# eth-cscs/conflux

Hardware: NVIDIA H100
Metric: LU GFLOP/s (FP64, (2/3)N^3) (higher is better)
Workload: dtype f64

## Files before the change

### conflux_b200/__init__.py

```python
import ctypes

import numpy as np

from ._lib import ConfluxError, LIB_PATH, SYMBOLS, ShareLayout, check, lib

__all__ = ["pinned_empty", "pinned_free", "Comm", "lu_params", "LU_rep", "LU_rep_fixed", "rbt_multipliers", "LU_rep_rbt", "lu_rbt_solve", "lu_rbt_apply_local", "residual", "validate", "lu_solve", "lu_rcond", "lu_refine", "lu_refine_x", "lu_equilibrate", "lu_svx", "lu_equilibrate_b", "lu_svxx", "lu_inverse", "lu_det", "rhs_local_cols", "lu_solve_local", "timeline", "auto_grid", "lu_dims", "init_matrix_host", "ConfluxError", "dbg", "cholesky", "chol_dims", "chol_auto_grid"]


def auto_grid(M, N, P):
    px, py, pz = ctypes.c_int(), ctypes.c_int(), ctypes.c_int()
    check(lib().cflx_auto_grid(int(M), int(N), int(P), ctypes.byref(px), ctypes.byref(py), ctypes.byref(pz)), "auto_grid")
    return px.value, py.value, pz.value


def lu_dims(M, N, v, Px, Py, Pz):
    o = (ctypes.c_int * 8)()
    check(lib().cflx_lu_dims(int(M), int(N), int(v), int(Px), int(Py), int(Pz), o), "lu_dims")
    return dict(M=o[0], N=o[1], Ml=o[2], Nl=o[3], Nt=o[4], nlayr=o[5], Mt=o[6], P=o[7])


def init_matrix_host(M, N, v, Px, Py, Pz, rank, seed=42, out=None):
    d = lu_dims(M, N, v, Px, Py, Pz)
    if out is None:
        out = np.empty((d["Ml"], d["Nl"]), dtype=np.float64)
# ... 816 lines not shown
                                 ctypes.byref(exp), ctypes.byref(neg), ctypes.byref(fz), ctypes.byref(nf)), "dbg_det")
        return dict(mantissa=mant.value, exponent=exp.value, neg=neg.value, first_zero=fz.value, nonfinite=nf.value)

    @staticmethod
    def panel(P, reps=1):
        P = np.ascontiguousarray(P, dtype=np.float64)
        n, v = P.shape
        perm = np.zeros(v, dtype=np.int32)
        A00 = np.zeros((v, v))
        LU = np.zeros((max(n, 1), v))
        ms = ctypes.c_double()
        check(lib().cflx_dbg_panel(n, v, P.ctypes.data, perm.ctypes.data, A00.ctypes.data, LU.ctypes.data, int(reps),
                                   ctypes.byref(ms)), "dbg_panel")
        return perm, A00, LU[:n], ms.value

    @staticmethod
    def trsm(A00, B=None, R=None, nb=0, ld=0):
        A00 = np.ascontiguousarray(A00, dtype=np.float64)
        v = A00.shape[0]
        X = Y = None
        n = B.shape[0] if B is not None else R.shape[1]
        if B is not None:
            B = np.ascontiguousarray(B, dtype=np.float64)
            X = np.empty_like(B)
        if R is not None:
            R = np.ascontiguousarray(R, dtype=np.float64)
            Y = np.empty_like(R)
        check(lib().cflx_dbg_trsm(n, v, int(nb), int(ld), A00.ctypes.data, B.ctypes.data if B is not None else None,
                                  X.ctypes.data if X is not None else None, R.ctypes.data if R is not None else None,
                                  Y.ctypes.data if Y is not None else None), "dbg_trsm")
        return X, Y

    @staticmethod
    def diag_inverse(A00, nb):
        A00 = np.ascontiguousarray(A00, dtype=np.float64)
        v = A00.shape[0]
        Uinv = np.empty((max(v // nb, 1), nb, nb))
        LinvT = np.empty_like(Uinv)
        check(lib().cflx_dbg_diag_inverse(v, int(nb), A00.ctypes.data, Uinv.ctypes.data, LinvT.ctypes.data), "dbg_diag_inverse")
        return Uinv, LinvT

    @staticmethod
    def potrf_tile(A, variant=0):
        A = np.ascontiguousarray(A, dtype=np.float64)
        v = A.shape[0]
        L = np.empty((v, v))
        LT = np.empty((v, v))
        info = ctypes.c_int()
        check(lib().cflx_dbg_potrf_tile(v, A.ctypes.data, L.ctypes.data, LT.ctypes.data, ctypes.byref(info), int(variant)),
              "dbg_potrf_tile")
        return L, LT, info.value

    @staticmethod
    def getrf_nopiv_tile(A, tiny=0.0, variant=0):
        A = np.ascontiguousarray(A, dtype=np.float64)
        v = A.shape[0]
        LU = np.empty((v, v))
        nrepl, info = ctypes.c_int(), ctypes.c_int()
        check(lib().cflx_dbg_getrf_nopiv_tile(v, A.ctypes.data, float(tiny), LU.ctypes.data, ctypes.byref(nrepl),
                                              ctypes.byref(info), int(variant)), "dbg_getrf_nopiv_tile")
        return LU, nrepl.value, info.value

    @staticmethod
    def ozaki_gemm(AT, B, C=None, reps=1, want_planes=False, row0=0, col0=0, max_ctas=0):
        AT = np.ascontiguousarray(AT, dtype=np.float64)
        B = np.ascontiguousarray(B, dtype=np.float64)
# ... 43 lines not shown
```

### conflux_b200/_lib.py

```python
import ctypes
import os

_HERE = os.path.dirname(os.path.abspath(__file__))
LIB_PATH = os.path.join(_HERE, "libconflux_b200.so")
_lib = None

c_double_p = ctypes.POINTER(ctypes.c_double)
c_int_p = ctypes.POINTER(ctypes.c_int)


class ConfluxError(RuntimeError):
    pass


class ShareLayout(ctypes.Structure):
    _fields_ = [(f, ctypes.c_int) for f in ("M", "v", "Kappa", "Ml", "Nl", "Px", "Py", "pi", "pj")]


SYMBOLS = [
    "cflx_last_error", "cflx_version", "cflx_device_count", "cflx_get_unique_id", "cflx_comm_create",
    "cflx_comm_barrier", "cflx_comm_destroy", "cflx_host_alloc", "cflx_host_free", "cflx_auto_grid", "cflx_lu_dims", "cflx_init_matrix_host",
    "cflx_lu_create", "cflx_lu_info", "cflx_lu_set_local", "cflx_lu_queue_next_local", "cflx_lu_factor", "cflx_lu_factor_fixed", "cflx_rbt_multipliers", "cflx_lu_rbt", "cflx_lu_rbt_solve", "cflx_lu_rbt_apply_local", "cflx_lu_get_factors",
    "cflx_lu_get_permutation", "cflx_lu_residual", "cflx_lu_validate", "cflx_lu_solve", "cflx_lu_solve_trans", "cflx_rhs_local_cols", "cflx_lu_solve_local", "cflx_lu_rcond", "cflx_lu_refine", "cflx_lu_refine_x", "cflx_lu_equilibrate", "cflx_lu_svx", "cflx_lu_equilibrate_b", "cflx_lu_svxx", "cflx_lu_inverse", "cflx_lu_det", "cflx_lu_launch_count", "cflx_lu_uses_ozaki", "cflx_lu_set_profiling", "cflx_lu_phase_ms", "cflx_lu_timeline",
    "cflx_lu_set_kernel_timing", "cflx_lu_trailing_stats", "cflx_lu_destroy", "cflx_chol_auto_grid", "cflx_chol_auto_tile", "cflx_chol_dims", "cflx_chol_init_matrix_host",
    "cflx_chol_create", "cflx_chol_info", "cflx_chol_set_local", "cflx_chol_factor", "cflx_chol_get_local", "cflx_chol_validate",
    "cflx_chol_solve", "cflx_chol_solve_local", "cflx_chol_rcond", "cflx_chol_refine", "cflx_chol_refine_x", "cflx_chol_equilibrate", "cflx_chol_svx", "cflx_chol_equilibrate_b", "cflx_chol_svxx", "cflx_chol_inverse", "cflx_chol_det", "cflx_chol_launch_count", "cflx_chol_destroy", "cflx_dbg_gemm_tn", "cflx_dbg_gemm_narrow", "cflx_dbg_gemm_narrow_tn", "cflx_dbg_gemm_narrow_window", "cflx_dbg_diag_solve", "cflx_dbg_residual", "cflx_dbg_residual_x", "cflx_dbg_equil", "cflx_dbg_growth_cols", "cflx_dbg_inverse_share", "cflx_dbg_solve_local_share", "cflx_dbg_norm_share", "cflx_dbg_rbt_share", "cflx_dbg_chol_validate_share", "cflx_dbg_lu_validate_share", "cflx_dbg_chol_gather_cols", "cflx_dbg_refine_assemble", "cflx_dbg_refine_columns", "cflx_dbg_det", "cflx_dbg_panel", "cflx_dbg_trsm", "cflx_dbg_diag_inverse", "cflx_dbg_potrf_tile", "cflx_dbg_getrf_nopiv_tile", "cflx_dbg_push_pivots", "cflx_dbg_ozaki_gemm", "cflx_dbg_wgmma_peak", "cflx_dbg_fp64_peak", "cflx_dbg_fp64_peak_ex",
]


def _preload_nccl():
    import sys
    for d in sys.path:
        cand = os.path.join(d, "nvidia", "nccl", "lib", "libnccl.so.2")
        if os.path.exists(cand):
            try:
                ctypes.CDLL(cand, mode=ctypes.RTLD_GLOBAL)
                return cand
            except OSError:
                pass
    return None


def lib():
    global _lib
    if _lib is None:
        if not os.path.exists(LIB_PATH):
            raise ConfluxError(
                f"{LIB_PATH} is missing: build it with `python -c 'import __graft_entry__ as g; g.build()'` "
                "(conflux_b200 has no CPU fallback)")
        _preload_nccl()
        L = ctypes.CDLL(LIB_PATH)
        L.cflx_last_error.restype = ctypes.c_char_p
        L.cflx_version.restype = ctypes.c_char_p
        L.cflx_comm_destroy.restype = None
        L.cflx_lu_destroy.restype = None
        L.cflx_comm_destroy.argtypes = [ctypes.c_void_p]
        L.cflx_lu_destroy.argtypes = [ctypes.c_void_p]
        L.cflx_comm_barrier.argtypes = [ctypes.c_void_p]
        L.cflx_comm_create.argtypes = [ctypes.c_int, ctypes.c_int, ctypes.c_void_p, ctypes.c_int,
# ... 77 lines not shown
                                                          c_double_p]
        L.cflx_dbg_gemm_narrow.argtypes = [ctypes.c_int] * 3 + [ctypes.c_void_p] * 3 + [ctypes.c_double] * 2 + [
            ctypes.c_void_p, ctypes.c_int, c_double_p]
        L.cflx_dbg_gemm_narrow_tn.argtypes = [ctypes.c_int] * 3 + [ctypes.c_void_p] * 3 + [ctypes.c_double] * 2 + [
            ctypes.c_void_p, ctypes.c_int, c_double_p]
        _blk = [ctypes.c_void_p, ctypes.c_int, ctypes.c_int64, ctypes.c_int, ctypes.c_int]
        L.cflx_dbg_gemm_narrow_window.argtypes = [ctypes.c_int] * 4 + _blk * 3 + [ctypes.c_double] * 2 + [
            ctypes.c_int, ctypes.c_void_p, ctypes.c_void_p]
        L.cflx_dbg_diag_solve.argtypes = [ctypes.c_int] * 4 + [ctypes.c_void_p, ctypes.c_int, ctypes.c_int64] + [
            ctypes.c_int] * 3 + [ctypes.c_void_p] * 3
        share = ctypes.POINTER(ShareLayout)
        L.cflx_dbg_residual.argtypes = [ctypes.c_int, share, ctypes.c_void_p, ctypes.c_int] + [ctypes.c_void_p] * 4 + [
            ctypes.c_int, c_double_p]
        L.cflx_dbg_residual_x.argtypes = [ctypes.c_int, share, ctypes.c_void_p, ctypes.c_int] + [
            ctypes.c_void_p] * 6 + [ctypes.c_int, c_double_p]
        L.cflx_dbg_equil.argtypes = [share] + [ctypes.c_void_p] * 3 + [ctypes.c_char, ctypes.c_int] + [
            ctypes.c_void_p] * 7
        L.cflx_dbg_growth_cols.argtypes = [ctypes.c_int, share, ctypes.c_int] + [ctypes.c_void_p] * 4
        L.cflx_dbg_inverse_share.argtypes = [ctypes.c_int, share] + [ctypes.c_int] * 3 + [
            ctypes.c_void_p, ctypes.c_int] + [ctypes.c_void_p] * 3 + [ctypes.c_int]
        L.cflx_dbg_solve_local_share.argtypes = [ctypes.c_int, share] + [ctypes.c_int] * 3 + [
            ctypes.c_void_p, ctypes.c_int] + [ctypes.c_void_p] * 3 + [ctypes.c_int]
        L.cflx_dbg_norm_share.argtypes = [ctypes.c_int, share] + [ctypes.c_void_p] * 2
        L.cflx_dbg_rbt_share.argtypes = [ctypes.c_int, share, ctypes.c_int] + [ctypes.c_void_p] * 2 + [
            ctypes.c_int, ctypes.c_void_p, ctypes.c_int]
        L.cflx_dbg_chol_validate_share.argtypes = [share, ctypes.c_void_p, ctypes.c_int] + [ctypes.c_void_p] * 2
        L.cflx_dbg_lu_validate_share.argtypes = [share, ctypes.c_void_p, ctypes.c_int] + [ctypes.c_void_p] * 2
        L.cflx_dbg_chol_gather_cols.argtypes = [share, ctypes.c_int] + [ctypes.c_void_p] * 2
        L.cflx_dbg_refine_assemble.argtypes = [ctypes.c_int] * 12 + [ctypes.c_void_p] * 6
        L.cflx_dbg_refine_columns.argtypes = [ctypes.c_int] * 3 + [ctypes.c_void_p] * 10
        L.cflx_dbg_det.argtypes = [ctypes.c_int] + [ctypes.c_void_p] * 3 + [ctypes.c_int] + [ctypes.c_void_p] * 5
        L.cflx_dbg_panel.argtypes = [ctypes.c_int, ctypes.c_int] + [ctypes.c_void_p] * 4 + [ctypes.c_int, c_double_p]
        L.cflx_dbg_trsm.argtypes = [ctypes.c_int] * 3 + [ctypes.c_int64] + [ctypes.c_void_p] * 5
        L.cflx_dbg_diag_inverse.argtypes = [ctypes.c_int, ctypes.c_int] + [ctypes.c_void_p] * 3
        L.cflx_dbg_potrf_tile.argtypes = [ctypes.c_int] + [ctypes.c_void_p] * 4 + [ctypes.c_int]
        L.cflx_dbg_getrf_nopiv_tile.argtypes = [ctypes.c_int, ctypes.c_void_p, ctypes.c_double] + [ctypes.c_void_p] * 3 + [
            ctypes.c_int]
        L.cflx_dbg_push_pivots.argtypes = [ctypes.c_int, ctypes.c_int, ctypes.c_void_p, ctypes.c_int, ctypes.c_void_p, ctypes.c_int,
                                           ctypes.c_void_p, ctypes.c_void_p]
        L.cflx_dbg_ozaki_gemm.argtypes = [ctypes.c_int] * 6 + [ctypes.c_void_p] * 8 + [ctypes.c_int, c_double_p, c_double_p]
        L.cflx_dbg_wgmma_peak.argtypes = [ctypes.c_int, c_double_p]
        L.cflx_dbg_fp64_peak.argtypes = [ctypes.c_int, c_double_p]
        L.cflx_dbg_fp64_peak_ex.argtypes = [ctypes.c_int, c_double_p, c_double_p]
        _lib = L
    return _lib


def check(rc, what=""):
    if rc != 0:
        msg = lib().cflx_last_error().decode(errors="replace")
        raise ConfluxError(f"{what} failed with status {rc}: {msg}")
```

### conflux_b200/csrc/dbg.cu

```cuda
#include <algorithm>
#include <climits>
#include <limits>
#include <vector>

#include "../../include/conflux_b200.h"
#include "common.cuh"
#include "kernels.h"
#include "lu_state.h"

using namespace cflx;

namespace {
int check_device() {
    int n = 0;
    if (cudaGetDeviceCount(&n) != cudaSuccess || n == 0) {
        cudaGetLastError();
        set_last_error("no CUDA device visible: conflux_b200 has no CPU fallback");
        return CFLX_ERR_NO_DEVICE;
    }
    return CFLX_OK;
}

enum : unsigned { TILED = 1, COVERED = 2, NONEMPTY = 4 };

// ... 828 lines not shown
        for (int j = 0; j < v; ++j) A00T[(size_t)j * v + i] = A00[(size_t)i * v + j];
    const size_t vv = (size_t)v * v, panel = (size_t)v * ld;
    DevBuf<> dA, dAT, dUinv, dLinvT;
    CFLX_TRY(stage(dA, vv, A00));
    CFLX_TRY(stage(dAT, vv, A00T.data()));
    CFLX_TRY(stage(dUinv, vv));
    CFLX_TRY(stage(dLinvT, vv));
    CFLX_TRY(launch_diag_inverses(dA.as<double>(), v, nb, dUinv.as<double>(), dLinvT.as<double>(), 0));
    if (B && X_out) {
        for (int r = 0; r < n; ++r)
            for (int c = 0; c < v; ++c) BT[(size_t)c * ld + r] = B[(size_t)r * v + c];
        DevBuf<> dP, dL;
        CFLX_TRY(stage(dP, panel, BT.data()));
        CFLX_TRY(stage(dL, panel));
        CFLX_CUDA(cudaMemset(dL.p, 0, 8 * panel));
        CFLX_TRY(trsm_right_upper_T(dA.as<double>(), dUinv.as<double>(), v, nb, dP.as<double>(), dL.as<double>(), ld, n, 0));
        CFLX_TRY(fetch(BT.data(), dL.p, panel));
        for (int r = 0; r < n; ++r)
            for (int c = 0; c < v; ++c) X_out[(size_t)r * v + c] = BT[(size_t)c * ld + r];
    }
    if (R && Y_out) {
        for (int i = 0; i < v; ++i)
            for (int c = 0; c < n; ++c) RT[(size_t)i * ld + c] = R[(size_t)i * n + c];
        DevBuf<> dR, dU;
        CFLX_TRY(stage(dR, panel, RT.data()));
        CFLX_TRY(stage(dU, panel));
        CFLX_CUDA(cudaMemset(dU.p, 0, 8 * panel));
        CFLX_TRY(trsm_left_lower_unit(dAT.as<double>(), dLinvT.as<double>(), v, nb, dR.as<double>(), dU.as<double>(), ld,
                                      (int)round_up(n, 2), 0));
        CFLX_TRY(fetch(RT.data(), dU.p, panel));
        for (int i = 0; i < v; ++i)
            for (int c = 0; c < n; ++c) Y_out[(size_t)i * n + c] = RT[(size_t)i * ld + c];
    }
    CFLX_CUDA(cudaDeviceSynchronize());
    return CFLX_OK;
}

int cflx_dbg_diag_inverse(int v, int nb, const double* A00, double* Uinv_out, double* LinvT_out) {
    CFLX_TRY(check_device());
    REFUSE_IF(v <= 0 || nb <= 0 || v % nb != 0);
    REFUSE_IF(!A00);
    const size_t vv = (size_t)v * v, blocks = (size_t)v * nb;
    DevBuf<> dA, dU, dL;
    CFLX_TRY(stage(dA, vv, A00));
    CFLX_TRY(stage(dU, blocks));
    CFLX_TRY(stage(dL, blocks));
    CFLX_TRY(launch_diag_inverses(dA.as<double>(), v, nb, dU.as<double>(), dL.as<double>(), 0));
    CFLX_TRY(fetch(Uinv_out, dU.p, blocks));
    CFLX_TRY(fetch(LinvT_out, dL.p, blocks));
    CFLX_CUDA(cudaDeviceSynchronize());
    return CFLX_OK;
}

int cflx_dbg_potrf_tile(int v, const double* A, double* L_out, double* LT_out, int* info_out, int variant) {
    CFLX_TRY(check_device());
    REFUSE_IF(!A);
    REFUSE_IF(variant < 0 || variant > 2);
    REFUSE_IF(v < 4 || v > 512 || (variant == 1 && v != 128) || (variant == 2 && potrf_tile_scratch(v) == 0));
    const size_t vv = (size_t)v * v;
    DevBuf<> dD, dUT, dUc, dQ, dinfo;
    CFLX_TRY(stage(dD, vv, A));
    CFLX_TRY(stage(dUT, vv));
    CFLX_TRY(stage(dUc, vv));
    CFLX_TRY(stage<int>(dinfo, 1));
    if (variant == 2) CFLX_TRY(stage(dQ, potrf_tile_scratch(v)));
    CFLX_CUDA(cudaMemset(dUT.p, 0, 8 * vv));
// ... 156 lines not shown
```

### conflux_b200/csrc/kernels.h

```cpp
#pragma once
#include <cuda_runtime.h>

#include <cstdint>
#include <memory>

#include "common.cuh"

namespace cflx {

struct GemmArgs {
    int M, N, K;
    const double* AT;
    int64_t ldat;
    const double* B;
    int64_t ldb;
    const double* C;
    int64_t ldc;
    double* D;
    int64_t ldd;
    double alpha, beta;
};
int gemm_tn_setup();
int launch_gemm_tn(const GemmArgs& g, cudaStream_t stream);

// ... 51 lines not shown
    int* rowsrc;
};
int launch_plan_moves(const int* gpivots, int v, int Px, int pi, int fnpr, int Ml, const int* igri, MovePlan plan,
                      cudaStream_t stream);
int launch_push_phase1(const double* A, int64_t lda, int ncols, int col_lo, MovePlan plan, int v, double* tmp,
                       double* a01raw, int64_t ld01, int c0, cudaStream_t stream);
int launch_push_phase2(double* A, int64_t lda, int ncols, int col_lo, MovePlan plan, int v, cudaStream_t stream);
int launch_push_phase3(double* A, int64_t lda, int ncols, int col_lo, int fnpr, MovePlan plan, int v,
                       const double* tmp, cudaStream_t stream);
int launch_update_gri(int* gri, int* gri_tmp, int* igri, const int* rowsrc, int fnpr, int Ml, int v, int Px,
                      cudaStream_t stream);
int launch_compact_panel(const double* PT, int64_t ldp, double* PT2, int64_t ldp2, const int* rowsrc, int fnpr_old,
                         const int* npiv, int Ml, int v, cudaStream_t stream);
int launch_store_u_rows(double* A, int64_t lda, int fnpr_old, MovePlan plan, const double* U, int64_t ldu, int c0,
                        int ncols, int v, cudaStream_t stream);
int launch_store_diag(double* A, int64_t lda, int fnpr_old, MovePlan plan, const double* A00, int loff, int v,
                      cudaStream_t stream);
int launch_split_factors(const double* F, int64_t ldf, int n, double* LT, double* U, cudaStream_t stream);
int launch_gather_perm_rows(const double* A, int64_t lda, const int* perm, int n, double* out, cudaStream_t stream);
constexpr int SUMSQ_PARTIALS = 1184;
int launch_sumsq(const double* X, int64_t count, double* out, double* partials, cudaStream_t stream);
int launch_sum_partials(const double* partials, int n, double* out, cudaStream_t stream);
int launch_fill(double* p, int64_t n, double val, cudaStream_t stream);
int launch_iota_gri(int* gri, int* igri, int Ml, int v, int Px, int pi, cudaStream_t stream);
int launch_pack_bcast(const double* A00, const int* tags, int v, double* buf, cudaStream_t stream);
int launch_unpack_bcast(const double* buf, int v, double* A00, double* A00T, int* gpivots, cudaStream_t stream);
int launch_record_pivots(const int* gpivots, int v, int* hist, int k, cudaStream_t stream);

int launch_diag_inverses(const double* A00, int v, int nb, double* Uinv, double* LinvT, cudaStream_t stream);
int trsm_right_upper_T(const double* A00, const double* Uinv, int v, int nb, double* PT, double* LT, int64_t ld,
                       int n, cudaStream_t stream);
int trsm_left_lower_unit(const double* A00T, const double* LinvT, int v, int nb, double* R, double* U, int64_t ld,
                         int n, cudaStream_t stream);

size_t potrf_tile_scratch(int v);
int potrf_setup(int v);
int potrf_tile(double* D, double* UT, double* Q, int* info, int col0, int v, cudaStream_t stream, int64_t* launches);
int potrf_block128(double* D, int ldd, double* UT, int ldu, double* Uc, int* info, int col0, cudaStream_t stream);

bool getrf_nopiv_blocked(int v);
size_t getrf_nopiv_scratch(int v, bool blocked);
int launch_getrf_nopiv_tile(const double* Bt, int v, double tiny, double* A, double* AT, const int* tags_in, int* tags_out,
                            int* rec, int col0, bool blocked, double* scratch, cudaStream_t stream, int64_t* launches);
int launch_fixed_locate(const int* rows, int v, int Px, int pi, int fnpr, int n_old, const int* igri, int* pos,
                        cudaStream_t stream);
int launch_fixed_info_operand(int* rec, cudaStream_t stream);

int launch_gather_rows(const double* A, int64_t lda, const int* src_rows, int nrows, int ncols, double* out,
                       cudaStream_t stream);

int launch_gemm_narrow(int M, int N, int K, const double* A, int64_t lda, const double* B, int64_t ldb, const double* C,
                       int64_t ldc, double* D, int64_t ldd, double alpha, double beta, cudaStream_t stream);
int launch_gemm_narrow_tn(int M, int N, int K, const double* AT, int64_t ldat, const double* B, int64_t ldb,
                          const double* C, int64_t ldc, double* D, int64_t ldd, double alpha, double beta,
                          cudaStream_t stream);

enum class ResidMode { NN, TN, SymLower };

}
```

### conflux_b200/csrc/lu.cu

```cuda
#include <algorithm>
#include <climits>
#include <cmath>
#include <cstdarg>
#include <cstdlib>
#include <cstring>
#include <random>
#include <string>
#include <vector>

#include <nvtx3/nvToolsExt.h>

#include "lu_state.h"

namespace cflx {
static thread_local char g_err[1024] = "";
void set_last_error(const char* fmt, ...) {
    va_list ap;
    va_start(ap, fmt);
    vsnprintf(g_err, sizeof(g_err), fmt, ap);
    va_end(ap);
}
}

using namespace cflx;
// ... 440 lines not shown
        if (on_col) {
            CFLX_TRY(launch_store_diag(lu->A11, Nl, fnpr_old, lu->plan, A00, loff, v, s));
            lu->launches++;
        }
        return CFLX_OK;
    };
    if (!split_u) CFLX_TRY(store_factors());
    int npiv = v;
    if (lu->fixed) {
        npiv = lu->fix_npiv[k];
    } else if (Px > 1) {
        CFLX_CUDA(cudaEventSynchronize(lu->ev_npiv));
        npiv = *lu->h_npiv;
    }
    if (npiv < 0 || npiv > v || fnpr_old + npiv > Ml) {
        set_last_error("step %d: inconsistent pivot count %d (fnpr %d, Ml %d)", k, npiv, fnpr_old, Ml);
        return CFLX_ERR_STATE;
    }
    fnpr = fnpr_old + npiv;
    const int n_act = Ml - fnpr;
    const int64_t ld2 = std::max<int64_t>(2, round_up(n_act, 2));
    if (on_col && layer0 && n_act > 0) {
        {
            PhaseTimer t(lu, RG_step4_reshuffling, s);
            CFLX_TRY(launch_compact_panel(fused_l ? lu->W : lu->PT, ldk, fused_l ? lu->LT : lu->PT2, ld2, lu->plan.rowsrc,
                                          fnpr_old, lu->plan.npiv, Ml, v, s));
            lu->launches++;
        }
        if (!fused_l) {
            PhaseTimer t(lu, RG_step4_dtrsm, s);
            CFLX_TRY(trsm_right_upper_T(A00, lu->Uinv, v, lu->nb, lu->PT2, lu->LT, ld2, n_act, s));
            lu->launches += 2 * (v / lu->nb) - 1;
        }
        PhaseTimer t(lu, RG_storingresults, s);
        CFLX_TRY(launch_store_panel_T(lu->A11, Nl, fnpr, loff, n_act, v, lu->LT, ld2, s));
        lu->launches++;
    }
    if (Py * Pz > 1 && n_act > 0) {
        PhaseTimer t(lu, RG_step4_comm, s);
        CFLX_NCCL(ncclBroadcast(lu->LT, lu->LT, (size_t)v * ld2, ncclDouble, pjk * Pz, lu->jk_comm.c, s));
    }
    const bool next_col = (k + 1 < lu->Nt) && (pj == (k + 1) % Py);
    CFLX_TRY(ozaki_planes_a(lu, n_act, ld2, s));
    if (n_act > 0) CFLX_TRY(ozaki_planes_b(lu, 0, split_u ? std::min(v, ncols) : ncols, ldu, s));
    if (next_col) {
        const int w = std::min(v, ncols);
        CFLX_TRY(trailing_gemm(lu, k, 0, fnpr, n_act, c0, w, ld2, ldu, 0, s));
        cudaStream_t side = (lu->prof_mode == 1) ? nullptr : lu->side.s;
        cudaStream_t sp = side ? side : s;
        if (side) {
            CFLX_CUDA(cudaEventRecord(lu->ev_fork, s));
            CFLX_CUDA(cudaStreamWaitEvent(sp, lu->ev_fork, 0));
        }
        CFLX_TRY(panel_phase(lu, k + 1, fnpr, sp));
        if (side) CFLX_CUDA(cudaEventRecord(lu->ev_join, sp));
        if (split_u) {
            PhaseTimer t(lu, RG_step5_dtrsm, s);
            CFLX_TRY(trsm_left_lower_unit(A00T, lu->LinvT, v, lu->nb, lu->A01raw + v, lu->U + v, ldu, ncols - v, s));
            lu->launches += 2 * (v / lu->nb) - 1;
        }
        if (split_u) CFLX_TRY(store_factors());
        if (split_u && n_act > 0) CFLX_TRY(ozaki_planes_b(lu, w, ncols - w, ldu, s));
        const int leave = (side && lu->use_ozaki) ? lu->pws.cta_cap : 0;
        CFLX_TRY(trailing_gemm(lu, k, 1, fnpr, n_act, c0 + w, ncols - w, ld2, ldu, w, s, leave > 0 ? lu->oz.sms - leave : 0));
        if (side) CFLX_CUDA(cudaStreamWaitEvent(s, lu->ev_join, 0));
    } else {
        CFLX_TRY(trailing_gemm(lu, k, 0, fnpr, n_act, c0, ncols, ld2, ldu, 0, s));
    }
    return CFLX_OK;
}

SolveFactor lu_solve_factor(cflx_lu* lu) { return SolveFactor{*lu, lu->Cbuf, lu->Ml, &lu->jk_comm, &lu->ik_comm, lu->Pz}; }

int lu_permutation(cflx_lu* lu, std::vector<int>* perm) {
    perm->resize(lu->M);
    CFLX_CUDA(cudaMemcpyAsync(perm->data(), lu->hist, sizeof(int) * lu->M, cudaMemcpyDeviceToHost, lu->comm->stream));
    CFLX_CUDA(cudaStreamSynchronize(lu->comm->stream));
    return CFLX_OK;
}

int lu_solve_prepare(cflx_lu* lu) {
    cudaStream_t s = lu->comm->stream;
    const int v = lu->v, Px = lu->Px, Ml = lu->Ml;
    std::vector<int> hist;
    CFLX_TRY(lu_permutation(lu, &hist));
    if (lu->pk == 0) {
        lu->sv.inv.reset();
        if (!lu->Cbuf) CFLX_TRY(lu->Cbuf.alloc((size_t)Ml * lu->Nl));
        int rc = redistribute_pivoted_rows(lu, hist, true, lu->A11, lu->Cbuf);
        lu->xbuf.reset();
        if (rc) return rc;
        CFLX_TRY(solve_inverses(&lu->sv, lu_solve_factor(lu), false));
        if (lu->pj == 0) {
            std::vector<int> rows(Ml, 0);
// ... 997 lines not shown
```

### conflux_b200/csrc/trsm.cu

```cuda
#include "common.cuh"
#include "kernels.h"

namespace cflx {
namespace {
template <int NB>
__global__ void __launch_bounds__(1024) diag_inverse_kernel(const double* __restrict__ A00, int v, double* __restrict__ Uinv,
                                                            double* __restrict__ LinvT) {
    constexpr int EPL = (NB + 31) / 32;
    extern __shared__ double S[];
    constexpr int LD = NB + 1;
    const int j = blockIdx.x;
    const int warp = threadIdx.x >> 5, lane = threadIdx.x & 31, nwarps = blockDim.x >> 5;
    const double* blk = A00 + (size_t)(j * NB) * v + j * NB;
    for (int e = threadIdx.x; e < NB * NB; e += blockDim.x) S[(e / NB) * LD + e % NB] = blk[(size_t)(e / NB) * v + e % NB];
    __syncthreads();
    double* out = (blockIdx.y == 0 ? Uinv : LinvT) + (size_t)j * NB * NB;
    const int cols_per = (NB + gridDim.z - 1) / gridDim.z;
    const int c_lo = blockIdx.z * cols_per, c_hi = min(NB, c_lo + cols_per);
    for (int c = c_lo + warp; c < c_hi; c += nwarps) {
        double x[EPL];
#pragma unroll
        for (int e = 0; e < EPL; ++e) x[e] = 0.0;
        if (blockIdx.y == 0) {
            const double xc = 1.0 / S[c * LD + c];
// ... 44 lines not shown
        }
    }
}

template <int NB>
int launch_diag_nb(const double* A00, int v, double* Uinv, double* LinvT, cudaStream_t stream) {
    constexpr size_t smem = (size_t)NB * (NB + 1) * sizeof(double);
    constexpr int CS = NB > 64 ? NB / 32 : 1;
    const int warps = NB < 32 ? NB : 32;
    static PerDeviceMax cfg;
    CFLX_CUDA(cfg.raise(smem, [&] {
        return cudaFuncSetAttribute(diag_inverse_kernel<NB>, cudaFuncAttributeMaxDynamicSharedMemorySize, (int)smem);
    }));
    diag_inverse_kernel<NB><<<dim3(v / NB, 2, CS), 32 * warps, smem, stream>>>(A00, v, Uinv, LinvT);
    CFLX_CUDA(cudaGetLastError());
    return CFLX_OK;
}
}

int launch_diag_inverses(const double* A00, int v, int nb, double* Uinv, double* LinvT, cudaStream_t stream) {
    switch (nb) {
        case 128: return launch_diag_nb<128>(A00, v, Uinv, LinvT, stream);
        case 64: return launch_diag_nb<64>(A00, v, Uinv, LinvT, stream);
        case 32: return launch_diag_nb<32>(A00, v, Uinv, LinvT, stream);
        case 16: return launch_diag_nb<16>(A00, v, Uinv, LinvT, stream);
        case 8: return launch_diag_nb<8>(A00, v, Uinv, LinvT, stream);
        case 4: return launch_diag_nb<4>(A00, v, Uinv, LinvT, stream);
        default:
            set_last_error("diag_inverses: unsupported block size %d", nb);
            return CFLX_ERR_UNSUPPORTED;
    }
}

int trsm_right_upper_T(const double* A00, const double* Uinv, int v, int nb, double* PT, double* LT, int64_t ld, int n,
                       cudaStream_t stream) {
    if (n <= 0) return CFLX_OK;
    const int nblk = v / nb;
    const int N = (n + 1) & ~1;
    for (int j = 0; j < nblk; ++j) {
        GemmArgs g{};
        g.M = nb; g.N = N; g.K = nb;
        g.AT = Uinv + (size_t)j * nb * nb; g.ldat = nb;
        g.B = PT + (int64_t)j * nb * ld; g.ldb = ld;
        g.C = nullptr; g.ldc = ld;
        g.D = LT + (int64_t)j * nb * ld; g.ldd = ld;
        g.alpha = 1.0; g.beta = 0.0;
        CFLX_TRY(launch_gemm_tn(g, stream));
        const int rest = v - (j + 1) * nb;
        if (rest > 0) {
            GemmArgs u{};
            u.M = rest; u.N = N; u.K = nb;
            u.AT = A00 + (size_t)(j * nb) * v + (j + 1) * nb; u.ldat = v;
            u.B = LT + (int64_t)j * nb * ld; u.ldb = ld;
            u.C = PT + (int64_t)(j + 1) * nb * ld; u.ldc = ld;
            u.D = PT + (int64_t)(j + 1) * nb * ld; u.ldd = ld;
            u.alpha = -1.0; u.beta = 1.0;
            CFLX_TRY(launch_gemm_tn(u, stream));
        }
    }
    return CFLX_OK;
}

int trsm_left_lower_unit(const double* A00T, const double* LinvT, int v, int nb, double* R, double* U, int64_t ld, int n,
                         cudaStream_t stream) {
    if (n <= 0) return CFLX_OK;
    const int nblk = v / nb;
    for (int j = 0; j < nblk; ++j) {
        GemmArgs g{};
        g.M = nb; g.N = n; g.K = nb;
        g.AT = LinvT + (size_t)j * nb * nb; g.ldat = nb;
        g.B = R + (int64_t)j * nb * ld; g.ldb = ld;
        g.C = nullptr; g.ldc = ld;
        g.D = U + (int64_t)j * nb * ld; g.ldd = ld;
        g.alpha = 1.0; g.beta = 0.0;
        CFLX_TRY(launch_gemm_tn(g, stream));
        const int rest = v - (j + 1) * nb;
        if (rest > 0) {
            GemmArgs u{};
            u.M = rest; u.N = n; u.K = nb;
            u.AT = A00T + (size_t)(j * nb) * v + (j + 1) * nb; u.ldat = v;
            u.B = U + (int64_t)j * nb * ld; u.ldb = ld;
            u.C = R + (int64_t)(j + 1) * nb * ld; u.ldc = ld;
            u.D = R + (int64_t)(j + 1) * nb * ld; u.ldd = ld;
            u.alpha = -1.0; u.beta = 1.0;
            CFLX_TRY(launch_gemm_tn(u, stream));
        }
    }
    return CFLX_OK;
}

}
```

### include/conflux_b200.h

```cpp
#ifndef CONFLUX_B200_H
#define CONFLUX_B200_H

#include <stddef.h>
#include <stdint.h>

#ifdef __cplusplus
extern "C" {
#endif

typedef enum {
    CFLX_OK = 0,
    CFLX_ERR_ARG = -1,
    CFLX_ERR_CUDA = -2,
    CFLX_ERR_NCCL = -3,
    CFLX_ERR_UNSUPPORTED = -4,
    CFLX_ERR_STATE = -5,
    CFLX_ERR_NO_DEVICE = -6
} cflx_status;

typedef struct cflx_comm cflx_comm;
typedef struct cflx_lu cflx_lu;

#define CFLX_UNIQUE_ID_BYTES 128

// ... 64 lines not shown
int cflx_chol_dims(int N, int v, int Px, int Py, int Pz, int* dims_out);
int cflx_chol_init_matrix_host(int N, int v, int Px, int Py, int Pz, int rank, double* local_out);
int cflx_chol_create(cflx_comm*, int N, int v, int Px, int Py, int Pz, cflx_chol** out);
int cflx_chol_info(const cflx_chol*, int* info_out);
int cflx_chol_set_local(cflx_chol*, const double* host_local);
int cflx_chol_factor(cflx_chol*, double* ms_out);
int cflx_chol_get_local(cflx_chol*, double* L_host);
int cflx_chol_validate(cflx_chol*, double* frob_abs_out, double* frob_rel_out);
int cflx_chol_solve(cflx_chol*, int nrhs, const double* B, int ldb, double* X, int ldx);
int cflx_chol_solve_local(cflx_chol*, int nrhs, const double* B_local, int ldb, double* X_local, int ldx);
int cflx_chol_rcond(cflx_chol*, double* rcond_out, double* anorm_out);
int cflx_chol_refine(cflx_chol*, int nrhs, const double* B, int ldb, double* X, int ldx, double* ferr_out,
                     double* berr_out);
int cflx_chol_refine_x(cflx_chol*, int nrhs, const double* B, int ldb, double* X, int ldx, double* rcond_out,
                       double* berr_out, double* err_bnds_norm_out, double* err_bnds_comp_out, int* info_out);
int cflx_chol_equilibrate(cflx_chol*, int apply, double* s_out, double* scond_out, double* amax_out, char* equed_out,
                          int* info_out);
int cflx_chol_svx(cflx_chol*, int nrhs, const double* B, int ldb, double* X, int ldx, double* rcond_out, double* ferr_out,
                  double* berr_out, char* equed_out, int* info_out);
int cflx_chol_equilibrate_b(cflx_chol*, int apply, double* s_out, double* scond_out, double* amax_out, char* equed_out,
                            int* info_out);
int cflx_chol_svxx(cflx_chol*, int nrhs, const double* B, int ldb, double* X, int ldx, double* rcond_out,
                   double* rpvgrw_out, double* berr_out, double* err_bnds_norm_out, double* err_bnds_comp_out,
                   char* equed_out, int* info_out);
int cflx_chol_inverse(cflx_chol*, double* Ainv_local);
int cflx_chol_det(cflx_chol*, int unscaled, double* logdet_out, double* mant_out, int64_t* exp_out);
int cflx_chol_launch_count(cflx_chol*, int64_t* count_out, int reset);
void cflx_chol_destroy(cflx_chol*);

int cflx_dbg_gemm_tn(int M, int N, int K, const double* AT, int at_rows, int64_t ldat, int64_t at_off, const double* B,
                     int b_rows, int64_t ldb, int64_t b_off, const double* C, int c_rows, int64_t ldc, int row_off,
                     int col_off, double alpha, double beta, int in_place, double* D_out, double* C_out, int reps,
                     double* ms_out);
int cflx_dbg_gemm_narrow(int M, int N, int K, const double* A, const double* B, const double* C, double alpha, double beta,
                         double* D, int reps, double* ms_out);
int cflx_dbg_gemm_narrow_tn(int M, int N, int K, const double* AT, const double* B, const double* C, double alpha,
                            double beta, double* D, int reps, double* ms_out);
int cflx_dbg_gemm_narrow_window(int trans, int M, int N, int K, const double* A, int a_rows, int64_t lda, int a_row,
                                int a_col, const double* B, int b_rows, int64_t ldb, int b_row, int b_col, const double* C,
                                int c_rows, int64_t ldc, int c_row, int c_col, double alpha, double beta, int in_place,
                                double* D_out, double* C_out);
int cflx_dbg_diag_solve(int tri, int lower, int v, int nb, const double* share, int rows, int64_t ld, int row0, int col0,
                        int ldn, const double* R, double* Y_out, double* inv_out);
typedef struct { int M, v, Kappa, Ml, Nl, Px, Py, pi, pj; } cflx_share_layout;
int cflx_dbg_residual(int mode, const cflx_share_layout* share, const double* A, int nrhs, const double* Xc,
                      const double* Xr, double* P_out, double* Q_out, int reps, double* ms_out);
int cflx_dbg_residual_x(int mode, const cflx_share_layout* share, const double* A, int nrhs, const double* Xc,
                        const double* Xct, const double* Xr, const double* Xrt, double* hi_out, double* lo_out, int reps,
                        double* ms_out);
int cflx_dbg_equil(const cflx_share_layout* share, const double* A, const double* r, const double* c, char equed, int ncols,
                   double* rowmax_out, double* colmax_out, double* diag_out, double* scaled_out, double* sym_scaled_out,
                   double* growth_out, int* zero_pivot_out);
int cflx_dbg_growth_cols(int mode, const cflx_share_layout* share, int ncols, const double* F, const double* A,
                         double* amax_out, double* fmax_out);
int cflx_dbg_inverse_share(int mode, const cflx_share_layout* share, int c0, int nc, int rows, const double* X, int ldx,
                           const int* perm, double* W_out, double* share_inout, int zero_fill);
int cflx_dbg_solve_local_share(int mode, const cflx_share_layout* share, int nrhs, int c0, int w, const double* B, int ldb,
                               double* Bk_out, const double* Xk, double* X_inout, int ldx);
int cflx_dbg_norm_share(int mode, const cflx_share_layout* share, const double* A, double* out);
int cflx_dbg_rbt_share(int op, const cflx_share_layout* share, int depth, const double* u, const double* v, int ncols,
                       double* share_inout, int ld);
int cflx_dbg_chol_validate_share(const cflx_share_layout* share, const double* A, int t, double* PT_out, double* sumsq_out);
int cflx_dbg_lu_validate_share(const cflx_share_layout* share, const double* C, int t, double* LT_out, double* U_out);
int cflx_dbg_chol_gather_cols(const cflx_share_layout* share, int gfirst, const double* pieces, double* Bc_out);
int cflx_dbg_refine_assemble(int mode, int Px, int Py, int Pz, int v, int M, int Ml, int Nl, int nn, int tn, int nrhs,
                             int ldn, const double* all, const double* B, double* R_out, double* ratio_out, double* W_out,
// ... 28 lines not shown
```

Measured before the change: 26470.

## Add small-grid warp-per-tile TRSM step kernel and defer L panel store

Merges the two blocked TRSM sweeps into one trsm_solve and adds a warp-per-16xCW-tile DMMA kernel. It is chosen when the step GEMMs are too small to fill the GPU, so those many small, latency-bound launches can spread across more SMs. Separately, when the next panel column is local, the L panel store moves after the next panel's TRSM so it stays off the critical path. A debug sweep entry point and Python binding are added; the risk is that the heuristic selects the slower path for some shapes.

```diff
diff --git a/conflux_b200/__init__.py b/conflux_b200/__init__.py
--- a/conflux_b200/__init__.py
+++ b/conflux_b200/__init__.py
@@ -872,6 +872,20 @@
         return X, Y
 
     @staticmethod
+    def trsm_sweep(off, inv, R, U, v, nb, n, r_off=(0, 0), right=False, path=0, reps=1):
+        off = np.ascontiguousarray(off, dtype=np.float64)
+        inv = np.ascontiguousarray(inv, dtype=np.float64)
+        R = np.ascontiguousarray(R, dtype=np.float64)
+        U0 = np.ascontiguousarray(U, dtype=np.float64)
+        assert off.shape == (v, v) and inv.size == v * nb and U0.shape == R.shape
+        Uout, Rout, ms = np.empty_like(R), np.empty_like(R), ctypes.c_double()
+        check(lib().cflx_dbg_trsm_sweep(1 if right else 0, int(v), int(nb), int(n), off.ctypes.data, inv.ctypes.data,
+                                        R.ctypes.data, R.shape[0], R.shape[1], int(r_off[0]), int(r_off[1]),
+                                        U0.ctypes.data, int(path), Uout.ctypes.data, Rout.ctypes.data, int(reps),
+                                        ctypes.byref(ms)), "dbg_trsm_sweep")
+        return Uout, Rout, ms.value
+
+    @staticmethod
     def diag_inverse(A00, nb):
         A00 = np.ascontiguousarray(A00, dtype=np.float64)
         v = A00.shape[0]
diff --git a/conflux_b200/_lib.py b/conflux_b200/_lib.py
--- a/conflux_b200/_lib.py
+++ b/conflux_b200/_lib.py
@@ -24,7 +24,7 @@
     "cflx_lu_get_permutation", "cflx_lu_residual", "cflx_lu_validate", "cflx_lu_solve", "cflx_lu_solve_trans", "cflx_rhs_local_cols", "cflx_lu_solve_local", "cflx_lu_rcond", "cflx_lu_refine", "cflx_lu_refine_x", "cflx_lu_equilibrate", "cflx_lu_svx", "cflx_lu_equilibrate_b", "cflx_lu_svxx", "cflx_lu_inverse", "cflx_lu_det", "cflx_lu_launch_count", "cflx_lu_uses_ozaki", "cflx_lu_set_profiling", "cflx_lu_phase_ms", "cflx_lu_timeline",
     "cflx_lu_set_kernel_timing", "cflx_lu_trailing_stats", "cflx_lu_destroy", "cflx_chol_auto_grid", "cflx_chol_auto_tile", "cflx_chol_dims", "cflx_chol_init_matrix_host",
     "cflx_chol_create", "cflx_chol_info", "cflx_chol_set_local", "cflx_chol_factor", "cflx_chol_get_local", "cflx_chol_validate",
-    "cflx_chol_solve", "cflx_chol_solve_local", "cflx_chol_rcond", "cflx_chol_refine", "cflx_chol_refine_x", "cflx_chol_equilibrate", "cflx_chol_svx", "cflx_chol_equilibrate_b", "cflx_chol_svxx", "cflx_chol_inverse", "cflx_chol_det", "cflx_chol_launch_count", "cflx_chol_destroy", "cflx_dbg_gemm_tn", "cflx_dbg_gemm_narrow", "cflx_dbg_gemm_narrow_tn", "cflx_dbg_gemm_narrow_window", "cflx_dbg_diag_solve", "cflx_dbg_residual", "cflx_dbg_residual_x", "cflx_dbg_equil", "cflx_dbg_growth_cols", "cflx_dbg_inverse_share", "cflx_dbg_solve_local_share", "cflx_dbg_norm_share", "cflx_dbg_rbt_share", "cflx_dbg_chol_validate_share", "cflx_dbg_lu_validate_share", "cflx_dbg_chol_gather_cols", "cflx_dbg_refine_assemble", "cflx_dbg_refine_columns", "cflx_dbg_det", "cflx_dbg_panel", "cflx_dbg_trsm", "cflx_dbg_diag_inverse", "cflx_dbg_potrf_tile", "cflx_dbg_getrf_nopiv_tile", "cflx_dbg_push_pivots", "cflx_dbg_ozaki_gemm", "cflx_dbg_wgmma_peak", "cflx_dbg_fp64_peak", "cflx_dbg_fp64_peak_ex",
+    "cflx_chol_solve", "cflx_chol_solve_local", "cflx_chol_rcond", "cflx_chol_refine", "cflx_chol_refine_x", "cflx_chol_equilibrate", "cflx_chol_svx", "cflx_chol_equilibrate_b", "cflx_chol_svxx", "cflx_chol_inverse", "cflx_chol_det", "cflx_chol_launch_count", "cflx_chol_destroy", "cflx_dbg_gemm_tn", "cflx_dbg_trsm_sweep", "cflx_dbg_gemm_narrow", "cflx_dbg_gemm_narrow_tn", "cflx_dbg_gemm_narrow_window", "cflx_dbg_diag_solve", "cflx_dbg_residual", "cflx_dbg_residual_x", "cflx_dbg_equil", "cflx_dbg_growth_cols", "cflx_dbg_inverse_share", "cflx_dbg_solve_local_share", "cflx_dbg_norm_share", "cflx_dbg_rbt_share", "cflx_dbg_chol_validate_share", "cflx_dbg_lu_validate_share", "cflx_dbg_chol_gather_cols", "cflx_dbg_refine_assemble", "cflx_dbg_refine_columns", "cflx_dbg_det", "cflx_dbg_panel", "cflx_dbg_trsm", "cflx_dbg_diag_inverse", "cflx_dbg_potrf_tile", "cflx_dbg_getrf_nopiv_tile", "cflx_dbg_push_pivots", "cflx_dbg_ozaki_gemm", "cflx_dbg_wgmma_peak", "cflx_dbg_fp64_peak", "cflx_dbg_fp64_peak_ex",
 ]
 
 
@@ -168,6 +168,8 @@
         L.cflx_dbg_det.argtypes = [ctypes.c_int] + [ctypes.c_void_p] * 3 + [ctypes.c_int] + [ctypes.c_void_p] * 5
         L.cflx_dbg_panel.argtypes = [ctypes.c_int, ctypes.c_int] + [ctypes.c_void_p] * 4 + [ctypes.c_int, c_double_p]
         L.cflx_dbg_trsm.argtypes = [ctypes.c_int] * 3 + [ctypes.c_int64] + [ctypes.c_void_p] * 5
+        L.cflx_dbg_trsm_sweep.argtypes = [ctypes.c_int] * 4 + [ctypes.c_void_p] * 3 + [ctypes.c_int, ctypes.c_int64] + [
+            ctypes.c_int] * 2 + [ctypes.c_void_p, ctypes.c_int] + [ctypes.c_void_p] * 2 + [ctypes.c_int, ctypes.c_void_p]
         L.cflx_dbg_diag_inverse.argtypes = [ctypes.c_int, ctypes.c_int] + [ctypes.c_void_p] * 3
         L.cflx_dbg_potrf_tile.argtypes = [ctypes.c_int] + [ctypes.c_void_p] * 4 + [ctypes.c_int]
         L.cflx_dbg_getrf_nopiv_tile.argtypes = [ctypes.c_int, ctypes.c_void_p, ctypes.c_double] + [ctypes.c_void_p] * 3 + [
diff --git a/conflux_b200/csrc/dbg.cu b/conflux_b200/csrc/dbg.cu
--- a/conflux_b200/csrc/dbg.cu
+++ b/conflux_b200/csrc/dbg.cu
@@ -884,6 +884,44 @@
         for (int i = 0; i < v; ++i)
             for (int c = 0; c < n; ++c) Y_out[(size_t)i * n + c] = RT[(size_t)i * ld + c];
     }
+    CFLX_CUDA(cudaDeviceSynchronize());
+    return CFLX_OK;
+}
+
+int cflx_dbg_trsm_sweep(int right, int v, int nb, int n, const double* off, const double* inv, const double* R, int r_rows,
+                        int64_t ld, int row_off, int col_off, const double* U0, int path, double* U_out, double* R_out,
+                        int reps, double* ms_out) {
+    CFLX_TRY(check_device());
+    REFUSE_IF(v <= 0 || nb <= 0 || n <= 0 || v % nb != 0);
+    REFUSE_IF(nb != 4 && nb != 8 && nb != 16 && nb != 32 && nb != 64 && nb != 128);
+    REFUSE_IF(path < 0 || path > 2);
+    REFUSE_IF(!off || !inv || !R || !U0);
+    REFUSE_IF(r_rows <= 0 || ld <= 0 || row_off < 0 || col_off < 0);
+    const int N = right ? (n + 1) & ~1 : n;
+    REFUSE_IF(row_off + v > r_rows || col_off + N > ld);
+    const size_t vv = (size_t)v * v, r_n = (size_t)r_rows * ld;
+    DevBuf<> dA, dI, dR, dR0, dU, dU0;
+    CFLX_TRY(stage(dA, vv, off));
+    CFLX_TRY(stage(dI, (size_t)v * nb, inv));
+    CFLX_TRY(stage(dR, r_n));
+    CFLX_TRY(stage(dR0, r_n, R));
+    CFLX_TRY(stage(dU, r_n));
+    CFLX_TRY(stage(dU0, r_n, U0));
+    auto restore = [&]() -> int {
+        CFLX_CUDA(cudaMemcpy(dR.p, dR0.p, sizeof(double) * r_n, cudaMemcpyDeviceToDevice));
+        CFLX_CUDA(cudaMemcpy(dU.p, dU0.p, sizeof(double) * r_n, cudaMemcpyDeviceToDevice));
+        return CFLX_OK;
+    };
+    const int64_t at = (int64_t)row_off * ld + col_off;
+    auto run = [&] {
+        return trsm_solve(dA.as<double>(), dI.as<double>(), v, nb, dR.as<double>() + at, dU.as<double>() + at, ld, N, path, 0);
+    };
+    CFLX_TRY(restore());
+    CFLX_TRY(time_reps(run, reps, ms_out));
+    CFLX_TRY(restore());
+    CFLX_TRY(run());
+    CFLX_TRY(fetch(U_out, dU.p, r_n));
+    CFLX_TRY(fetch(R_out, dR.p, r_n));
     CFLX_CUDA(cudaDeviceSynchronize());
     return CFLX_OK;
 }
diff --git a/conflux_b200/csrc/kernels.h b/conflux_b200/csrc/kernels.h
--- a/conflux_b200/csrc/kernels.h
+++ b/conflux_b200/csrc/kernels.h
@@ -107,6 +107,8 @@
                        int n, cudaStream_t stream);
 int trsm_left_lower_unit(const double* A00T, const double* LinvT, int v, int nb, double* R, double* U, int64_t ld,
                          int n, cudaStream_t stream);
+int trsm_solve(const double* off, const double* inv, int v, int nb, double* R, double* U, int64_t ld, int N, int path,
+               cudaStream_t stream);
 
 size_t potrf_tile_scratch(int v);
 int potrf_setup(int v);
diff --git a/conflux_b200/csrc/lu.cu b/conflux_b200/csrc/lu.cu
--- a/conflux_b200/csrc/lu.cu
+++ b/conflux_b200/csrc/lu.cu
@@ -496,15 +496,20 @@
             CFLX_TRY(trsm_right_upper_T(A00, lu->Uinv, v, lu->nb, lu->PT2, lu->LT, ld2, n_act, s));
             lu->launches += 2 * (v / lu->nb) - 1;
         }
+    }
+    const bool next_col = (k + 1 < lu->Nt) && (pj == (k + 1) % Py);
+    auto store_l = [&]() -> int {
+        if (!(on_col && layer0 && n_act > 0)) return CFLX_OK;
         PhaseTimer t(lu, RG_storingresults, s);
         CFLX_TRY(launch_store_panel_T(lu->A11, Nl, fnpr, loff, n_act, v, lu->LT, ld2, s));
         lu->launches++;
-    }
+        return CFLX_OK;
+    };
+    if (!next_col) CFLX_TRY(store_l());
     if (Py * Pz > 1 && n_act > 0) {
         PhaseTimer t(lu, RG_step4_comm, s);
         CFLX_NCCL(ncclBroadcast(lu->LT, lu->LT, (size_t)v * ld2, ncclDouble, pjk * Pz, lu->jk_comm.c, s));
     }
-    const bool next_col = (k + 1 < lu->Nt) && (pj == (k + 1) % Py);
     CFLX_TRY(ozaki_planes_a(lu, n_act, ld2, s));
     if (n_act > 0) CFLX_TRY(ozaki_planes_b(lu, 0, split_u ? std::min(v, ncols) : ncols, ldu, s));
     if (next_col) {
@@ -524,6 +529,7 @@
             lu->launches += 2 * (v / lu->nb) - 1;
         }
         if (split_u) CFLX_TRY(store_factors());
+        CFLX_TRY(store_l());
         if (split_u && n_act > 0) CFLX_TRY(ozaki_planes_b(lu, w, ncols - w, ldu, s));
         const int leave = (side && lu->use_ozaki) ? lu->pws.cta_cap : 0;
         CFLX_TRY(trailing_gemm(lu, k, 1, fnpr, n_act, c0 + w, ncols - w, ld2, ldu, w, s, leave > 0 ? lu->oz.sms - leave : 0));
diff --git a/conflux_b200/csrc/trsm.cu b/conflux_b200/csrc/trsm.cu
--- a/conflux_b200/csrc/trsm.cu
+++ b/conflux_b200/csrc/trsm.cu
@@ -100,61 +100,137 @@
     }
 }
 
-int trsm_right_upper_T(const double* A00, const double* Uinv, int v, int nb, double* PT, double* LT, int64_t ld, int n,
-                       cudaStream_t stream) {
-    if (n <= 0) return CFLX_OK;
+namespace {
+constexpr int STEP_WARPS = 8;
+
+template <int NT, int KB>
+__device__ __forceinline__ void step_mma(double (&acc)[NT][4], const double* __restrict__ AT, int64_t lda, int M, int m0,
+                                         const double* __restrict__ B, int64_t ldb, int ncol, int K, int lane) {
+    const int g = lane >> 2, t = lane & 3;
+    const bool r0 = m0 + g < M, r1 = m0 + 8 + g < M;
+#pragma unroll
+    for (int j = 0; j < NT; ++j) acc[j][0] = acc[j][1] = acc[j][2] = acc[j][3] = 0.0;
+    const int nks = (K + 7) / 8;
+    for (int kb = 0; kb < nks; kb += KB) {
+        double a[KB][4];
+#pragma unroll
+        for (int s = 0; s < KB; ++s) {
+            const int k = 8 * (kb + s) + t;
+            const bool lo = kb + s < nks, hi = lo && 8 * (kb + s) + 4 < K;
+            const double* p = AT + (int64_t)k * lda + m0 + g;
+            a[s][0] = lo && r0 ? __ldg(p) : 0.0;
+            a[s][1] = lo && r1 ? __ldg(p + 8) : 0.0;
+            a[s][2] = hi && r0 ? __ldg(p + 4 * lda) : 0.0;
+            a[s][3] = hi && r1 ? __ldg(p + 4 * lda + 8) : 0.0;
+        }
+#pragma unroll
+        for (int s = 0; s < KB; ++s) {
+            if (kb + s < nks) {
+                const int k = 8 * (kb + s) + t;
+                const bool hi = 8 * (kb + s) + 4 < K;
+#pragma unroll
+                for (int j = 0; j < NT; ++j) {
+                    const int c = 8 * j + g;
+                    double b[2];
+                    b[0] = c < ncol ? __ldg(B + (int64_t)k * ldb + c) : 0.0;
+                    b[1] = hi && c < ncol ? __ldg(B + (int64_t)(k + 4) * ldb + c) : 0.0;
+                    dmma16x8x8(acc[j], a[s], b);
+                }
+            }
+        }
+    }
+}
+
+template <int NT>
+__global__ void __launch_bounds__(32 * STEP_WARPS, 2) trsm_step_kernel(GemmArgs g) {
+    constexpr int CW = 8 * NT, KB = NT >= 4 ? 4 : 8;
+    const int warp = threadIdx.x >> 5, lane = threadIdx.x & 31, gq = lane >> 2, t = lane & 3;
+    const int mt = (g.M + 15) / 16, ct = (g.N + CW - 1) / CW;
+    const int64_t task = (int64_t)blockIdx.x * STEP_WARPS + warp;
+    if (task >= (int64_t)mt * ct) return;
+    const int m0 = 16 * (int)(task % mt), c0 = CW * (int)(task / mt);
+    double acc[NT][4];
+    step_mma<NT, KB>(acc, g.AT, g.ldat, g.M, m0, g.B + c0, g.ldb, g.N - c0, g.K, lane);
+    const bool use_c = (g.beta != 0.0);
+#pragma unroll
+    for (int j = 0; j < NT; ++j)
+#pragma unroll
+        for (int e = 0; e < 4; ++e) {
+            const int r = m0 + gq + 8 * (e >> 1), c = c0 + 8 * j + 2 * t + (e & 1);
+            if (r < g.M && c < g.N) {
+                const double cv = use_c ? g.C[(int64_t)r * g.ldc + c] : 0.0;
+                g.D[(int64_t)r * g.ldd + c] = fma(g.alpha, acc[j][e], g.beta * cv);
+            }
+        }
+}
+
+int sm_count(int* sms) {
+    int dev = 0;
+    CFLX_CUDA(cudaGetDevice(&dev));
+    CFLX_CUDA(cudaDeviceGetAttribute(sms, cudaDevAttrMultiProcessorCount, dev));
+    return CFLX_OK;
+}
+
+int launch_trsm_step(const GemmArgs& g, int sms, cudaStream_t stream) {
+    if (g.M <= 0 || g.N <= 0 || g.K <= 0) return CFLX_OK;
+    const int64_t mt = (g.M + 15) / 16;
+    auto ctas = [&](int cw) { return (mt * ((g.N + cw - 1) / cw) + STEP_WARPS - 1) / STEP_WARPS; };
+    const int64_t wave = 2 * (int64_t)sms;
+    if (ctas(8) <= wave) trsm_step_kernel<1><<<(unsigned)ctas(8), 32 * STEP_WARPS, 0, stream>>>(g);
+    else if (ctas(16) <= wave) trsm_step_kernel<2><<<(unsigned)ctas(16), 32 * STEP_WARPS, 0, stream>>>(g);
+    else trsm_step_kernel<4><<<(unsigned)ctas(32), 32 * STEP_WARPS, 0, stream>>>(g);
+    CFLX_CUDA(cudaGetLastError());
+    return CFLX_OK;
+}
+
+bool trsm_use_steps(int v, int nb, int n, int sms) {
+    const int64_t m = v - nb > nb ? v - nb : nb;
+    return (m + 15) / 16 * ((n + 7) / 8) <= (int64_t)2 * sms * STEP_WARPS;
+}
+
+}
+
+int trsm_solve(const double* off, const double* inv, int v, int nb, double* R, double* U, int64_t ld, int N, int path,
+               cudaStream_t stream) {
+    if (N <= 0) return CFLX_OK;
+    int sms = 0;
+    CFLX_TRY(sm_count(&sms));
+    const bool steps = path == 1 || (path == 0 && trsm_use_steps(v, nb, N, sms)) || (N & 1);
+    auto launch = [&](const GemmArgs& g) { return steps ? launch_trsm_step(g, sms, stream) : launch_gemm_tn(g, stream); };
     const int nblk = v / nb;
-    const int N = (n + 1) & ~1;
     for (int j = 0; j < nblk; ++j) {
         GemmArgs g{};
         g.M = nb; g.N = N; g.K = nb;
-        g.AT = Uinv + (size_t)j * nb * nb; g.ldat = nb;
-        g.B = PT + (int64_t)j * nb * ld; g.ldb = ld;
+        g.AT = inv + (size_t)j * nb * nb; g.ldat = nb;
+        g.B = R + (int64_t)j * nb * ld; g.ldb = ld;
         g.C = nullptr; g.ldc = ld;
-        g.D = LT + (int64_t)j * nb * ld; g.ldd = ld;
+        g.D = U + (int64_t)j * nb * ld; g.ldd = ld;
         g.alpha = 1.0; g.beta = 0.0;
-        CFLX_TRY(launch_gemm_tn(g, stream));
+        CFLX_TRY(launch(g));
         const int rest = v - (j + 1) * nb;
         if (rest > 0) {
             GemmArgs u{};
             u.M = rest; u.N = N; u.K = nb;
-            u.AT = A00 + (size_t)(j * nb) * v + (j + 1) * nb; u.ldat = v;
-            u.B = LT + (int64_t)j * nb * ld; u.ldb = ld;
-            u.C = PT + (int64_t)(j + 1) * nb * ld; u.ldc = ld;
-            u.D = PT + (int64_t)(j + 1) * nb * ld; u.ldd = ld;
-            u.alpha = -1.0; u.beta = 1.0;
-            CFLX_TRY(launch_gemm_tn(u, stream));
-        }
-    }
-    return CFLX_OK;
-}
-
-int trsm_left_lower_unit(const double* A00T, const double* LinvT, int v, int nb, double* R, double* U, int64_t ld, int n,
-                         cudaStream_t stream) {
-    if (n <= 0) return CFLX_OK;
-    const int nblk = v / nb;
-    for (int j = 0; j < nblk; ++j) {
-        GemmArgs g{};
-        g.M = nb; g.N = n; g.K = nb;
-        g.AT = LinvT + (size_t)j * nb * nb; g.ldat = nb;
-        g.B = R + (int64_t)j * nb * ld; g.ldb = ld;
-        g.C = nullptr; g.ldc = ld;
-        g.D = U + (int64_t)j * nb * ld; g.ldd = ld;
-        g.alpha = 1.0; g.beta = 0.0;
-        CFLX_TRY(launch_gemm_tn(g, stream));
-        const int rest = v - (j + 1) * nb;
-        if (rest > 0) {
-            GemmArgs u{};
-            u.M = rest; u.N = n; u.K = nb;
-            u.AT = A00T + (size_t)(j * nb) * v + (j + 1) * nb; u.ldat = v;
+            u.AT = off + (size_t)(j * nb) * v + (j + 1) * nb; u.ldat = v;
             u.B = U + (int64_t)j * nb * ld; u.ldb = ld;
             u.C = R + (int64_t)(j + 1) * nb * ld; u.ldc = ld;
             u.D = R + (int64_t)(j + 1) * nb * ld; u.ldd = ld;
             u.alpha = -1.0; u.beta = 1.0;
-            CFLX_TRY(launch_gemm_tn(u, stream));
-        }
-    }
-    return CFLX_OK;
-}
-
-}
+            CFLX_TRY(launch(u));
+        }
+    }
+    return CFLX_OK;
+}
+
+int trsm_right_upper_T(const double* A00, const double* Uinv, int v, int nb, double* PT, double* LT, int64_t ld, int n,
+                       cudaStream_t stream) {
+    if (n <= 0) return CFLX_OK;
+    return trsm_solve(A00, Uinv, v, nb, PT, LT, ld, (n + 1) & ~1, 0, stream);
+}
+
+int trsm_left_lower_unit(const double* A00T, const double* LinvT, int v, int nb, double* R, double* U, int64_t ld, int n,
+                         cudaStream_t stream) {
+    return trsm_solve(A00T, LinvT, v, nb, R, U, ld, n, 0, stream);
+}
+
+}
diff --git a/include/conflux_b200.h b/include/conflux_b200.h
--- a/include/conflux_b200.h
+++ b/include/conflux_b200.h
@@ -120,6 +120,9 @@
                      int b_rows, int64_t ldb, int64_t b_off, const double* C, int c_rows, int64_t ldc, int row_off,
                      int col_off, double alpha, double beta, int in_place, double* D_out, double* C_out, int reps,
                      double* ms_out);
+int cflx_dbg_trsm_sweep(int right, int v, int nb, int n, const double* off, const double* inv, const double* R, int r_rows,
+                        int64_t ld, int row_off, int col_off, const double* U0, int path, double* U_out, double* R_out,
+                        int reps, double* ms_out);
 int cflx_dbg_gemm_narrow(int M, int N, int K, const double* A, const double* B, const double* C, double alpha, double beta,
                          double* D, int reps, double* ms_out);
 int cflx_dbg_gemm_narrow_tn(int M, int N, int K, const double* AT, const double* B, const double* C, double alpha,
```

New measurement: 26680 (median of 6 runs). Within noise of the previous version (+0.8%).
